# SHI-Labs/Versatile-Diffusion

Hardware: NVIDIA H100
Metric: 512x512 images/sec @ 50-step DDIM (bs=4/GPU) (higher is better)
Workload: dtype bf16

## Files before the change

versatile-diffusion_b200/csrc/attention.cu:

```cuda
#include "common.cuh"
#include "host_util.h"

namespace vdb {

constexpr int kBQ = 128;
constexpr float kRescaleThreshold = 8.0f;

struct alignas(64) AttnParams {
  CUtensorMap tmQ;
  CUtensorMap tmK;
  CUtensorMap tmV;
  int Nq, Nk;
  int q_bs, kv_bs;
  int q_col0, k_col0;
  int dv;
  int causal;
  float scale_log2;
  __nv_bfloat16* out;
  long long ldo;
  const int* kv_len;
};

template <int DK, int DVP, int BKV, int KV_STAGES>
constexpr size_t attention_smem_bytes() {
  return (DK / 64) * kBQ * 128 + KV_STAGES * ((DK / 64) * BKV * 128 + (BKV / 64) * DVP * 128) + (1 + 4 * KV_STAGES) * 8 + 1024;
}

template <int DK, int DVP, int BKV, int KV_STAGES, bool VARLEN = false>
__global__ void __launch_bounds__(288, 1) attention_kernel(const __grid_constant__ AttnParams p) {
  constexpr int KA = DK / 64;
  constexpr int KVA = BKV / 64;
  constexpr uint32_t kQBytes = KA * kBQ * 128;
  constexpr uint32_t kKBytes = KA * BKV * 128;
  constexpr uint32_t kVAtom = DVP * 128;
  constexpr uint32_t kVBytes = KVA * kVAtom;
  static_assert(BKV == 64 || BKV == 128, "kv tile");
  static_assert(kVAtom % 1024 == 0, "V atom must keep 1024B alignment");
  static_assert(DVP % 16 == 0 && DVP <= 256, "invalid wgmma N for PV");

  extern __shared__ __align__(1024) uint8_t smem_raw[];
  uint8_t* smem = reinterpret_cast<uint8_t*>((reinterpret_cast<uintptr_t>(smem_raw) + 1023) & ~uintptr_t(1023));
  uint8_t* sQ = smem;
  uint8_t* sK = sQ + kQBytes;
  uint8_t* sV = sK + KV_STAGES * kKBytes;
  uint64_t* q_full = reinterpret_cast<uint64_t*>(sV + KV_STAGES * kVBytes);
  uint64_t* k_full = q_full + 1;
  uint64_t* k_empty = k_full + KV_STAGES;
  uint64_t* v_full = k_empty + KV_STAGES;
  uint64_t* v_empty = v_full + KV_STAGES;

  const int warp = threadIdx.x >> 5;
  const int lane = threadIdx.x & 31;
  const int q0 = blockIdx.x * kBQ;
  const int head = blockIdx.y;
  const int b = blockIdx.z;

  int nk = 0;
  int ntiles = (p.Nk + BKV - 1) / BKV;
  if (p.causal) ntiles = min(ntiles, (q0 + kBQ + BKV - 1) / BKV);

  if (warp == 8 && lane == 0) {
    tma_prefetch_desc(&p.tmQ);
    tma_prefetch_desc(&p.tmK);
    tma_prefetch_desc(&p.tmV);
  }
  if (threadIdx.x == 0) {
    mbar_init(q_full, 1);
    for (int s = 0; s < KV_STAGES; ++s) {
      mbar_init(&k_full[s], 1); mbar_init(&k_empty[s], 8);
      mbar_init(&v_full[s], 1); mbar_init(&v_empty[s], 8);
    }
    fence_barrier_init();
  }
  __syncthreads();
  pdl_launch_dependents();
  pdl_wait();
  if constexpr (VARLEN) {
    nk = max(0, min(p.kv_len[b], p.Nk));
    ntiles = (nk + BKV - 1) / BKV;
  }

  if (warp == 8) {
    if (lane == 0) {
      mbar_arrive_expect_tx(q_full, kQBytes);
      for (int a = 0; a < KA; ++a)
        tma_load_2d(sQ + a * kBQ * 128, &p.tmQ, q_full, p.q_col0 + head * DK + a * 64, b * p.q_bs + q0);
      for (int j = 0; j < ntiles; ++j) {
        const int st = j % KV_STAGES;
        const uint32_t ph = (j / KV_STAGES) & 1;
        mbar_wait(&k_empty[st], ph ^ 1);
        mbar_arrive_expect_tx(&k_full[st], kKBytes);
        for (int a = 0; a < KA; ++a)
          tma_load_2d(sK + st * kKBytes + a * BKV * 128, &p.tmK, &k_full[st], p.k_col0 + head * DK + a * 64,
                      b * p.kv_bs + j * BKV);
        mbar_wait(&v_empty[st], ph ^ 1);
        mbar_arrive_expect_tx(&v_full[st], kVBytes);
        for (int a = 0; a < KVA; ++a)
          tma_load_2d(sV + st * kVBytes + a * kVAtom, &p.tmV, &v_full[st], b * p.kv_bs + j * BKV + a * 64, head * DVP);
      }
    }
    return;
  }

  const int g = warp >> 2;
  const int row0 = g * 64 + (warp & 3) * 16 + (lane >> 2);
  const int c2 = 2 * (lane & 3);
  const int q_idx[2] = {q0 + row0, q0 + row0 + 8};
  const int ksteps = (p.dv + 15) / 16;
  float o[DVP / 2];
#pragma unroll
  for (int i = 0; i < DVP / 2; ++i) o[i] = 0.f;
  float m_ref[2] = {-INFINITY, -INFINITY};
  float l_sum[2] = {0.f, 0.f};
  mbar_wait(q_full, 0);
#pragma unroll 1
  for (int j = 0; j < ntiles; ++j) {
    const int st = j % KV_STAGES;
    const uint32_t ph = (j / KV_STAGES) & 1;
    float s[BKV / 2];
    mbar_wait(&k_full[st], ph);
    wgmma_fence();
#pragma unroll
    for (int a = 0; a < KA; ++a) {
      const uint64_t qd = make_desc_sw128(smem_u32(sQ + a * kBQ * 128 + g * 64 * 128));
      const uint64_t kd = make_desc_sw128(smem_u32(sK + st * kKBytes + a * BKV * 128));
#pragma unroll
      for (int k = 0; k < 4; ++k)
        if (a * 4 + k < ksteps)
          wgmma_ss<BKV>(s, qd + 2 * k, kd + 2 * k, (a > 0 || k > 0) ? 1u : 0u);
    }
    wgmma_commit();
    wgmma_wait<0>();
    wgmma_fence_regs(s);
    __syncwarp();
    if (lane == 0) mbar_arrive(&k_empty[st]);

    const int kv0 = j * BKV;
    if (kv0 + BKV > (VARLEN ? nk : p.Nk) || p.causal) {
#pragma unroll
      for (int i = 0; i < 2; ++i) {
        const int lim = p.causal ? min(p.Nk, q_idx[i] + 1) : (VARLEN ? nk : p.Nk);
#pragma unroll
        for (int jj = 0; jj < BKV / 8; ++jj)
#pragma unroll
          for (int e = 0; e < 2; ++e)
            if (kv0 + 8 * jj + c2 + e >= lim) s[4 * jj + 2 * i + e] = -INFINITY;
      }
    }
    float m_scaled[2];
#pragma unroll
    for (int i = 0; i < 2; ++i) {
      float mx = -INFINITY;
#pragma unroll
      for (int jj = 0; jj < BKV / 8; ++jj) mx = fmaxf(mx, fmaxf(s[4 * jj + 2 * i], s[4 * jj + 2 * i + 1]));
      mx = fmaxf(mx, __shfl_xor_sync(0xffffffffu, mx, 1));
      mx = fmaxf(mx, __shfl_xor_sync(0xffffffffu, mx, 2));
      const float m_new = fmaxf(m_ref[i], mx);
      if (j == 0 || m_ref[i] == -INFINITY) {
        m_ref[i] = m_new;
      } else if ((m_new - m_ref[i]) * p.scale_log2 > kRescaleThreshold) {
        const float factor = ex2_mufu((m_ref[i] - m_new) * p.scale_log2);
        m_ref[i] = m_new;
        l_sum[i] *= factor;
#pragma unroll
        for (int jj = 0; jj < DVP / 8; ++jj) {
          o[4 * jj + 2 * i] *= factor;
          o[4 * jj + 2 * i + 1] *= factor;
        }
      }
      m_scaled[i] = (m_ref[i] == -INFINITY) ? 0.f : m_ref[i] * p.scale_log2;
    }
    uint32_t pa[BKV / 16][4];
#pragma unroll
    for (int kk = 0; kk < BKV / 16; ++kk) {
#pragma unroll
      for (int h = 0; h < 4; ++h) {
        const int i = h & 1;
        const int idx = 8 * kk + 4 * (h >> 1) + 2 * i;
        const float e0 = ex2_mufu(fmaf(s[idx], p.scale_log2, -m_scaled[i]));
        const float e1 = ex2_mufu(fmaf(s[idx + 1], p.scale_log2, -m_scaled[i]));
        l_sum[i] += e0 + e1;
        pa[kk][h] = pack_bf16x2(e0, e1);
      }
    }
    mbar_wait(&v_full[st], ph);
    wgmma_fence();
#pragma unroll
    for (int kk = 0; kk < BKV / 16; ++kk) {
      const uint64_t vd = make_desc_sw128(smem_u32(sV + st * kVBytes + (kk >> 2) * kVAtom));
      wgmma_rs<DVP>(o, pa[kk], vd + 2 * (kk & 3), 1u);
    }
    wgmma_commit();
    wgmma_wait<0>();
    wgmma_fence_regs(o);
    __syncwarp();
    if (lane == 0) mbar_arrive(&v_empty[st]);
  }

#pragma unroll
  for (int i = 0; i < 2; ++i) {
    float l = l_sum[i];
    l += __shfl_xor_sync(0xffffffffu, l, 1);
    l += __shfl_xor_sync(0xffffffffu, l, 2);
    const float inv_l = (VARLEN && !(l > 0.f)) ? 0.f : 1.f / l;
    if (q_idx[i] >= p.Nq) continue;
    __nv_bfloat16* orow = p.out + (static_cast<long long>(b) * p.q_bs + q_idx[i]) * p.ldo + head * p.dv;
#pragma unroll
    for (int jj = 0; jj < DVP / 8; ++jj) {
      const int col = 8 * jj + c2;
      if (col < p.dv)
        *reinterpret_cast<uint32_t*>(orow + col) = pack_bf16x2(o[4 * jj + 2 * i] * inv_l, o[4 * jj + 2 * i + 1] * inv_l);
    }
  }
}

struct AttnArgs {
  const void *Q, *K, *Vt;
  long long ldq, ldk, ldv;
  int B, H, q_bstride, kv_bstride;
};

template <int DK, int DVP, int BKV, int KV_STAGES, bool VARLEN = false>
static int launch_attention(AttnParams& p, const AttnArgs& a, cudaStream_t stream) {
  constexpr size_t smem = attention_smem_bytes<DK, DVP, BKV, KV_STAGES>();
  static_assert(smem <= 227 * 1024, "attention smem budget");
  auto kernel = attention_kernel<DK, DVP, BKV, KV_STAGES, VARLEN>;
  static bool configured = false;
  if (!configured) {
    VDB_CUDA_CHECK(cudaFuncSetAttribute(kernel, cudaFuncAttributeMaxDynamicSharedMemorySize, static_cast<int>(smem)));
    prefer_max_smem(kernel);
    configured = true;
  }
  int rc = make_tmap_2d(&p.tmQ, a.Q, static_cast<uint64_t>(a.ldq), static_cast<uint64_t>(a.B) * a.q_bstride, a.ldq * 2, 64, kBQ);
  if (rc) return rc;
  rc = make_tmap_2d(&p.tmK, a.K, static_cast<uint64_t>(a.ldk), static_cast<uint64_t>(a.B) * a.kv_bstride, a.ldk * 2, 64, BKV);
  if (rc) return rc;
  rc = make_tmap_2d(&p.tmV, a.Vt, static_cast<uint64_t>(a.B) * a.kv_bstride, static_cast<uint64_t>(a.H) * DVP, a.ldv * 2, 64, DVP);
  if (rc) return rc;
  dim3 grid((p.Nq + kBQ - 1) / kBQ, a.H, a.B);
  VDB_CUDA_CHECK(launch_pdl(kernel, grid, dim3(288), smem, stream, p));
  count_launch();
  return VDB_OK;
}

}

using namespace vdb;

extern "C" {

int vdb_attention_dk_pad(int d_head) { return d_head <= 64 ? 64 : (d_head <= 128 ? 128 : (d_head <= 192 ? 192 : -1)); }
int vdb_attention_dv_pad(int d_head) {
  if (d_head <= 48) return 48;
  if (d_head <= 64) return 64;
  if (d_head <= 80) return 80;
  if (d_head <= 160) return 160;
  return -1;
}

static int attention_prepare(const void* Q, long long ldq, int q_col0, const void* K, long long ldk, int k_col0, const void* Vt,
                             long long ldv, void* out, long long ldo, int B, int H, int Nq, int Nk, int q_bstride, int kv_bstride,
                             int d_head, float scale, int causal, AttnParams& p, AttnArgs& a) {
  if (!Q || !K || !Vt || !out || B <= 0 || H <= 0 || Nq <= 0 || Nk <= 0)
    return set_error(VDB_ERR_INVALID, "attention: null/empty argument");
  const int DK = vdb_attention_dk_pad(d_head), DVP = vdb_attention_dv_pad(d_head);
  if (DK < 0 || DVP < 0) return set_error(VDB_ERR_UNSUPPORTED, "attention: d_head %d not supported (<= 160)", d_head);
  if ((d_head % 8) || (ldo % 8) || (ldq % 8) || (ldk % 8) || (ldv % 8))
    return set_error(VDB_ERR_INVALID, "attention: d_head and leading dims must be multiples of 8");
  if (q_bstride <= 0) q_bstride = Nq;
  if (kv_bstride <= 0) kv_bstride = Nk;
  if (q_bstride < Nq || kv_bstride < Nk || (kv_bstride % 8))
    return set_error(VDB_ERR_INVALID, "attention: need q_bstride >= Nq, kv_bstride >= Nk and kv_bstride %% 8 == 0 (got %d, %d)",
                     q_bstride, kv_bstride);
  memset(&p, 0, sizeof(p));
  a = AttnArgs{Q, K, Vt, ldq, ldk, ldv, B, H, q_bstride, kv_bstride};
  p.Nq = Nq; p.Nk = Nk; p.q_bs = q_bstride; p.kv_bs = kv_bstride; p.q_col0 = q_col0; p.k_col0 = k_col0; p.dv = d_head; p.causal = causal;
  p.scale_log2 = scale * 1.4426950408889634f;
  p.out = reinterpret_cast<__nv_bfloat16*>(out);
  p.ldo = ldo;
  return VDB_OK;
}

int vdb_attention_bf16(const void* Q, long long ldq, int q_col0, const void* K, long long ldk, int k_col0,
                       const void* Vt, long long ldv, void* out, long long ldo, int B, int H, int Nq, int Nk,
                       int q_bstride, int kv_bstride, int d_head, float scale, int causal, void* stream) {
  AttnParams p;
  AttnArgs a{};
  const int rc = attention_prepare(Q, ldq, q_col0, K, ldk, k_col0, Vt, ldv, out, ldo, B, H, Nq, Nk, q_bstride, kv_bstride, d_head,
                                   scale, causal, p, a);
  if (rc) return rc;
  const int DK = vdb_attention_dk_pad(d_head), DVP = vdb_attention_dv_pad(d_head);
  cudaStream_t st = reinterpret_cast<cudaStream_t>(stream);
  if (DK == 64 && DVP == 48) return launch_attention<64, 48, 128, 2>(p, a, st);
  if (DK == 64 && DVP == 64) return launch_attention<64, 64, 128, 2>(p, a, st);
  if (DK == 128 && DVP == 80) return launch_attention<128, 80, 128, 2>(p, a, st);
  if (DK == 192 && DVP == 160) return launch_attention<192, 160, 64, 2>(p, a, st);
  return set_error(VDB_ERR_UNSUPPORTED, "attention: no kernel for d_head %d", d_head);
}

int vdb_attention_varlen_bf16(const void* Q, long long ldq, int q_col0, const void* K, long long ldk, int k_col0,
                              const void* Vt, long long ldv, void* out, long long ldo, int B, int H, int Nq, int Nk,
                              int q_bstride, int kv_bstride, int d_head, float scale, int causal, const int* kv_len,
                              void* stream) {
  if (!kv_len || (reinterpret_cast<uintptr_t>(kv_len) & 3))
    return set_error(VDB_ERR_INVALID, "attention_varlen: kv_len must be a non-null, 4-byte aligned device int32 [B]");
  if (causal) return set_error(VDB_ERR_INVALID, "attention_varlen: causal masking together with kv_len is not supported");
  if (vdb_attention_dk_pad(d_head) != 64 || vdb_attention_dv_pad(d_head) != 64)
    return set_error(VDB_ERR_UNSUPPORTED, "attention_varlen: only d_head 64 (BERT) is instantiated, got %d", d_head);
  AttnParams p;
  AttnArgs a{};
  const int rc = attention_prepare(Q, ldq, q_col0, K, ldk, k_col0, Vt, ldv, out, ldo, B, H, Nq, Nk, q_bstride, kv_bstride, d_head,
                                   scale, causal, p, a);
  if (rc) return rc;
  p.kv_len = kv_len;
  return launch_attention<64, 64, 128, 2, true>(p, a, reinterpret_cast<cudaStream_t>(stream));
}

}
```

versatile-diffusion_b200/csrc/common.cuh:

```cuda
#pragma once
#include <cuda.h>
#include <cuda_bf16.h>
#include <cuda_runtime.h>
#include <stdint.h>

namespace vdb {

#define VDB_DEVINL __device__ __forceinline__

enum : int {
  VDB_OK = 0,
  VDB_ERR_INVALID = 1,
  VDB_ERR_CUDA = 2,
  VDB_ERR_UNSUPPORTED = 3,
};

VDB_DEVINL float4 lds_f4(uint32_t addr) {
  float4 v;
  asm volatile("ld.shared.v4.f32 {%0, %1, %2, %3}, [%4];" : "=f"(v.x), "=f"(v.y), "=f"(v.z), "=f"(v.w) : "r"(addr));
  return v;
}

VDB_DEVINL float2 lds_f2(uint32_t addr) {
  float2 v;
  asm volatile("ld.shared.v2.f32 {%0, %1}, [%2];" : "=f"(v.x), "=f"(v.y) : "r"(addr));
  return v;
}
VDB_DEVINL void stmatrix_x4(uint32_t addr, uint32_t r0, uint32_t r1, uint32_t r2, uint32_t r3) {
  asm volatile("stmatrix.sync.aligned.m8n8.x4.shared.b16 [%0], {%1, %2, %3, %4};" ::"r"(addr), "r"(r0), "r"(r1), "r"(r2), "r"(r3)
               : "memory");
}

VDB_DEVINL uint32_t smem_u32(const void* p) {
  return static_cast<uint32_t>(__cvta_generic_to_shared(p));
}

VDB_DEVINL uint32_t lane_id() {
  uint32_t l;
  asm volatile("mov.u32 %0, %%laneid;" : "=r"(l));
  return l;
}

VDB_DEVINL bool elect_one() {
  uint32_t pred = 0;
  asm volatile(
      "{\n\t"
      ".reg .pred P;\n\t"
      "elect.sync _|P, 0xffffffff;\n\t"
      "selp.u32 %0, 1, 0, P;\n\t"
      "}\n"
      : "=r"(pred));
  return pred != 0;
}

VDB_DEVINL void mbar_init(uint64_t* bar, uint32_t count) {
  asm volatile("mbarrier.init.shared::cta.b64 [%0], %1;" ::"r"(smem_u32(bar)), "r"(count));
}
VDB_DEVINL void fence_barrier_init() {
  asm volatile("fence.mbarrier_init.release.cluster;" ::: "memory");
}
VDB_DEVINL void fence_proxy_async_smem() {
  asm volatile("fence.proxy.async.shared::cta;" ::: "memory");
}
VDB_DEVINL void mbar_arrive_expect_tx(uint64_t* bar, uint32_t bytes) {
  asm volatile("mbarrier.arrive.expect_tx.shared::cta.b64 _, [%0], %1;" ::"r"(smem_u32(bar)),
               "r"(bytes)
               : "memory");
}
VDB_DEVINL void mbar_arrive(uint64_t* bar) {
  asm volatile("mbarrier.arrive.shared::cta.b64 _, [%0];" ::"r"(smem_u32(bar)) : "memory");
}
VDB_DEVINL bool mbar_try_wait(uint64_t* bar, uint32_t parity) {
  uint32_t ok;
  asm volatile(
      "{\n\t"
      ".reg .pred P;\n\t"
      "mbarrier.try_wait.parity.shared::cta.b64 P, [%1], %2;\n\t"
      "selp.u32 %0, 1, 0, P;\n\t"
      "}\n"
      : "=r"(ok)
      : "r"(smem_u32(bar)), "r"(parity)
      : "memory");
  return ok != 0;
}
VDB_DEVINL void mbar_wait(uint64_t* bar, uint32_t parity) {
  while (!mbar_try_wait(bar, parity)) {
  }
}

VDB_DEVINL void tma_prefetch_desc(const CUtensorMap* m) {
  asm volatile("prefetch.tensormap [%0];" ::"l"(reinterpret_cast<uint64_t>(m)) : "memory");
}
VDB_DEVINL void tma_load_2d(void* smem_dst, const CUtensorMap* m, uint64_t* bar, int c0, int c1) {
  asm volatile(
      "cp.async.bulk.tensor.2d.shared::cluster.global.tile.mbarrier::complete_tx::bytes"
      " [%0], [%1, {%3, %4}], [%2];" ::"r"(smem_u32(smem_dst)),
      "l"(reinterpret_cast<uint64_t>(m)), "r"(smem_u32(bar)), "r"(c0), "r"(c1)
      : "memory");
}
VDB_DEVINL void tma_load_4d(void* smem_dst, const CUtensorMap* m, uint64_t* bar, int c0, int c1,
                            int c2, int c3) {
  asm volatile(
      "cp.async.bulk.tensor.4d.shared::cluster.global.tile.mbarrier::complete_tx::bytes"
      " [%0], [%1, {%3, %4, %5, %6}], [%2];" ::"r"(smem_u32(smem_dst)),
      "l"(reinterpret_cast<uint64_t>(m)), "r"(smem_u32(bar)), "r"(c0), "r"(c1), "r"(c2), "r"(c3)
      : "memory");
}

VDB_DEVINL void tma_store_4d(const CUtensorMap* m, const void* smem_src, int c0, int c1, int c2, int c3) {
  asm volatile(
      "cp.async.bulk.tensor.4d.global.shared::cta.tile.bulk_group [%0, {%2, %3, %4, %5}], [%1];" ::"l"(
          reinterpret_cast<uint64_t>(m)),
      "r"(smem_u32(smem_src)), "r"(c0), "r"(c1), "r"(c2), "r"(c3)
      : "memory");
}
VDB_DEVINL void bulk_commit() { asm volatile("cp.async.bulk.commit_group;" ::: "memory"); }
template <int N>
VDB_DEVINL void bulk_wait_read() { asm volatile("cp.async.bulk.wait_group.read %0;" ::"n"(N) : "memory"); }
template <int N>
VDB_DEVINL void bulk_wait() { asm volatile("cp.async.bulk.wait_group %0;" ::"n"(N) : "memory"); }

VDB_DEVINL uint32_t cluster_ctarank() {
  uint32_t r;
  asm volatile("mov.u32 %0, %%cluster_ctarank;" : "=r"(r));
  return r;
}
VDB_DEVINL void cluster_sync_all() {
  asm volatile("barrier.cluster.arrive.release.aligned;\n\tbarrier.cluster.wait.acquire.aligned;" ::: "memory");
}
VDB_DEVINL uint32_t mapa_u32(uint32_t local_addr, uint32_t rank) {
  uint32_t r;
  asm volatile("mapa.shared::cluster.u32 %0, %1, %2;" : "=r"(r) : "r"(local_addr), "r"(rank));
  return r;
}
VDB_DEVINL void mbar_arrive_cluster(uint32_t cluster_addr) {
  asm volatile("mbarrier.arrive.release.cluster.shared::cluster.b64 _, [%0];" ::"r"(cluster_addr) : "memory");
}

VDB_DEVINL uint64_t make_desc_sw128(uint32_t smem_addr) {
  uint64_t d = 0;
  d |= static_cast<uint64_t>((smem_addr & 0x3FFFF) >> 4);
  d |= static_cast<uint64_t>(1) << 16;
  d |= static_cast<uint64_t>(1024 >> 4) << 32;
  d |= static_cast<uint64_t>(1) << 62;
  return d;
}
VDB_DEVINL void wgmma_fence() { asm volatile("wgmma.fence.sync.aligned;" ::: "memory"); }
VDB_DEVINL void wgmma_commit() { asm volatile("wgmma.commit_group.sync.aligned;" ::: "memory"); }
template <int N>
VDB_DEVINL void wgmma_wait() { asm volatile("wgmma.wait_group.sync.aligned %0;" ::"n"(N) : "memory"); }
template <int R>
VDB_DEVINL void wgmma_fence_regs(float (&d)[R]) {
#pragma unroll
  for (int i = 0; i < R; ++i) asm volatile("" : "+f"(d[i])::"memory");
}

VDB_DEVINL unsigned long long gtime() {
  unsigned long long t;
  asm volatile("mov.u64 %0, %%globaltimer;" : "=l"(t));
  return t;
}

VDB_DEVINL void pdl_wait() { asm volatile("griddepcontrol.wait;" ::: "memory"); }
VDB_DEVINL void pdl_launch_dependents() { asm volatile("griddepcontrol.launch_dependents;" ::: "memory"); }

VDB_DEVINL uint32_t pack_bf16x2(float lo, float hi) {
  __nv_bfloat162 v = __floats2bfloat162_rn(lo, hi);
  return *reinterpret_cast<uint32_t*>(&v);
}
VDB_DEVINL float2 unpack_bf16x2(uint32_t u) {
  __nv_bfloat162 v = *reinterpret_cast<__nv_bfloat162*>(&u);
  return __bfloat1622float2(v);
}
VDB_DEVINL float ex2_mufu(float x) {
  float y;
  asm("ex2.approx.ftz.f32 %0, %1;" : "=f"(y) : "f"(x));
  return y;
}
VDB_DEVINL float ex2_poly(float x) {
  x = fmaxf(x, -126.0f);
  const float r = x + 12582912.0f;
  const float f = x - (r - 12582912.0f);
  float p = fmaf(0.0550886838f, f, 0.242604051f);
  p = fmaf(p, f, 0.693276242f);
  p = fmaf(p, f, 0.99992894f);
  return __int_as_float(__float_as_int(p) + (__float_as_int(r) << 23));
}
VDB_DEVINL float silu_f(float x) { return __fdividef(x, 1.0f + __expf(-x)); }
VDB_DEVINL float silu_bf16_f(float x) {
  float th;
  asm("tanh.approx.f32 %0, %1;" : "=f"(th) : "f"(0.5f * x));
  const float hx = 0.5f * x;
  return fmaf(hx, th, hx);
}
VDB_DEVINL float gelu_erf_f(float x) { return 0.5f * x * (1.0f + erff(x * 0.70710678118654752f)); }
VDB_DEVINL float gelu_as_f(float x) {
  const float z = fabsf(x) * 0.70710678118654752f;
  const float t = __fdividef(1.0f, fmaf(0.3275911f, z, 1.0f));
  float poly = fmaf(1.061405429f, t, -1.453152027f);
  poly = fmaf(poly, t, 1.421413741f);
  poly = fmaf(poly, t, -0.284496736f);
  poly = fmaf(poly, t, 0.254829592f);
  const float erf_abs = 1.0f - poly * t * __expf(-z * z);
  return 0.5f * x * (1.0f + copysignf(erf_abs, x));
}
VDB_DEVINL float gelu_fast_f(float x) {
  const float u = x * fmaf(0.0356774081f, x * x, 0.7978845608f);
  float th;
  asm("tanh.approx.f32 %0, %1;" : "=f"(th) : "f"(u));
  const float hx = 0.5f * x;
  return fmaf(hx, th, hx);
}
VDB_DEVINL float quick_gelu_f(float x) { return __fdividef(x, 1.0f + __expf(-1.702f * x)); }

}

#include "wgmma.cuh"
```

Before: 4.652.

## Pipeline QK and PV wgmma across tiles with warp-specialized register reallocation

Restructures the attention consumer loop so the S=QK^T wgmma for tile j is issued together with the PV wgmma for tile j-1, with softmax overlapping the in-flight PV. The kernel grows to 384 threads: a 128-thread producer warpgroup gives up registers via setmaxnreg and two consumer warpgroups take more. It also adds a mask-free fast path for full tiles, offloads part of the exp2 work to an FMA polynomial for the DK=64/DVP=48 case, and fixes underflow handling in ex2_poly. The aim is to hide tensor-core latency behind softmax work, at the cost of higher register pressure and double-buffered P fragments. The QK k-step count is now fixed at DVP/16 instead of derived from p.dv, which looks like a semantic change.

```diff
diff --git a/versatile-diffusion_b200/csrc/attention.cu b/versatile-diffusion_b200/csrc/attention.cu
--- a/versatile-diffusion_b200/csrc/attention.cu
+++ b/versatile-diffusion_b200/csrc/attention.cu
@@ -1,3 +1,5 @@
+#include <type_traits>
+
 #include "common.cuh"
 #include "host_util.h"
 
@@ -5,6 +7,9 @@
 
 constexpr int kBQ = 128;
 constexpr float kRescaleThreshold = 8.0f;
+constexpr int kAttnThreads = 384;
+constexpr int kProducerRegs = 40;
+constexpr int kConsumerRegs = 232;
 
 struct alignas(64) AttnParams {
   CUtensorMap tmQ;
@@ -26,8 +31,12 @@
   return (DK / 64) * kBQ * 128 + KV_STAGES * ((DK / 64) * BKV * 128 + (BKV / 64) * DVP * 128) + (1 + 4 * KV_STAGES) * 8 + 1024;
 }
 
+__host__ __device__ constexpr int attention_exp2_poly_of8(int DK, int DVP) {
+  return (DK == 64 && DVP == 48) ? 1 : 0;
+}
+
 template <int DK, int DVP, int BKV, int KV_STAGES, bool VARLEN = false>
-__global__ void __launch_bounds__(288, 1) attention_kernel(const __grid_constant__ AttnParams p) {
+__global__ void __launch_bounds__(kAttnThreads, 1) attention_kernel(const __grid_constant__ AttnParams p) {
   constexpr int KA = DK / 64;
   constexpr int KVA = BKV / 64;
   constexpr uint32_t kQBytes = KA * kBQ * 128;
@@ -37,6 +46,8 @@
   static_assert(BKV == 64 || BKV == 128, "kv tile");
   static_assert(kVAtom % 1024 == 0, "V atom must keep 1024B alignment");
   static_assert(DVP % 16 == 0 && DVP <= 256, "invalid wgmma N for PV");
+  constexpr int kExp2PolyOf8 = attention_exp2_poly_of8(DK, DVP);
+  constexpr int kSSteps = DVP / 16;
 
   extern __shared__ __align__(1024) uint8_t smem_raw[];
   uint8_t* smem = reinterpret_cast<uint8_t*>((reinterpret_cast<uintptr_t>(smem_raw) + 1023) & ~uintptr_t(1023));
@@ -55,11 +66,7 @@
   const int head = blockIdx.y;
   const int b = blockIdx.z;
 
-  int nk = 0;
-  int ntiles = (p.Nk + BKV - 1) / BKV;
-  if (p.causal) ntiles = min(ntiles, (q0 + kBQ + BKV - 1) / BKV);
-
-  if (warp == 8 && lane == 0) {
+  if (warp == 0 && lane == 0) {
     tma_prefetch_desc(&p.tmQ);
     tma_prefetch_desc(&p.tmK);
     tma_prefetch_desc(&p.tmV);
@@ -75,13 +82,16 @@
   __syncthreads();
   pdl_launch_dependents();
   pdl_wait();
-  if constexpr (VARLEN) {
-    nk = max(0, min(p.kv_len[b], p.Nk));
-    ntiles = (nk + BKV - 1) / BKV;
-  }
-
-  if (warp == 8) {
-    if (lane == 0) {
+  auto key_count = [&] { return VARLEN ? max(0, min(p.kv_len[b], p.Nk)) : p.Nk; };
+  auto tile_count = [&](int nk) {
+    const int n = (nk + BKV - 1) / BKV;
+    return p.causal ? min(n, (q0 + kBQ + BKV - 1) / BKV) : n;
+  };
+
+  if (warp < 4) {
+    setmaxnreg_dec<kProducerRegs>();
+    const int ntiles = tile_count(key_count());
+    if (warp == 0 && lane == 0) {
       mbar_arrive_expect_tx(q_full, kQBytes);
       for (int a = 0; a < KA; ++a)
         tma_load_2d(sQ + a * kBQ * 128, &p.tmQ, q_full, p.q_col0 + head * DK + a * 64, b * p.q_bs + q0);
@@ -102,23 +112,26 @@
     return;
   }
 
-  const int g = warp >> 2;
+  setmaxnreg_inc<kConsumerRegs>();
+  const int nk = key_count();
+  const int ntiles = tile_count(nk);
+  const int g = (warp >> 2) - 1;
   const int row0 = g * 64 + (warp & 3) * 16 + (lane >> 2);
   const int c2 = 2 * (lane & 3);
   const int q_idx[2] = {q0 + row0, q0 + row0 + 8};
-  const int ksteps = (p.dv + 15) / 16;
   float o[DVP / 2];
 #pragma unroll
   for (int i = 0; i < DVP / 2; ++i) o[i] = 0.f;
   float m_ref[2] = {-INFINITY, -INFINITY};
   float l_sum[2] = {0.f, 0.f};
-  mbar_wait(q_full, 0);
-#pragma unroll 1
-  for (int j = 0; j < ntiles; ++j) {
+  float o_factor[2];
+  bool o_rescale[2];
+  float s[BKV / 2];
+  uint32_t pa[BKV / 16][4], pb[BKV / 16][4];
+
+  auto issue_s = [&](int j) {
     const int st = j % KV_STAGES;
-    const uint32_t ph = (j / KV_STAGES) & 1;
-    float s[BKV / 2];
-    mbar_wait(&k_full[st], ph);
+    mbar_wait(&k_full[st], (j / KV_STAGES) & 1);
     wgmma_fence();
 #pragma unroll
     for (int a = 0; a < KA; ++a) {
@@ -126,75 +139,126 @@
       const uint64_t kd = make_desc_sw128(smem_u32(sK + st * kKBytes + a * BKV * 128));
 #pragma unroll
       for (int k = 0; k < 4; ++k)
-        if (a * 4 + k < ksteps)
+        if (a * 4 + k < kSSteps)
           wgmma_ss<BKV>(s, qd + 2 * k, kd + 2 * k, (a > 0 || k > 0) ? 1u : 0u);
     }
     wgmma_commit();
-    wgmma_wait<0>();
-    wgmma_fence_regs(s);
+  };
+  auto issue_pv = [&](int j, const uint32_t(&pp)[BKV / 16][4]) {
+    const int st = j % KV_STAGES;
+    mbar_wait(&v_full[st], (j / KV_STAGES) & 1);
+    wgmma_fence();
+#pragma unroll
+    for (int kk = 0; kk < BKV / 16; ++kk) {
+      const uint64_t vd = make_desc_sw128(smem_u32(sV + st * kVBytes + (kk >> 2) * kVAtom));
+      wgmma_rs<DVP>(o, pp[kk], vd + 2 * (kk & 3), 1u);
+    }
+    wgmma_commit();
+  };
+  auto release = [&](uint64_t* empty, int j) {
     __syncwarp();
-    if (lane == 0) mbar_arrive(&k_empty[st]);
-
+    if (lane == 0) mbar_arrive(&empty[j % KV_STAGES]);
+  };
+  auto softmax_tile = [&](int j, uint32_t(&pp)[BKV / 16][4], auto masked) {
+    constexpr bool kMasked = decltype(masked)::value;
     const int kv0 = j * BKV;
-    if (kv0 + BKV > (VARLEN ? nk : p.Nk) || p.causal) {
-#pragma unroll
-      for (int i = 0; i < 2; ++i) {
-        const int lim = p.causal ? min(p.Nk, q_idx[i] + 1) : (VARLEN ? nk : p.Nk);
-#pragma unroll
-        for (int jj = 0; jj < BKV / 8; ++jj)
-#pragma unroll
-          for (int e = 0; e < 2; ++e)
-            if (kv0 + 8 * jj + c2 + e >= lim) s[4 * jj + 2 * i + e] = -INFINITY;
-      }
-    }
+    int lim[2];
+#pragma unroll
+    for (int i = 0; i < 2; ++i) lim[i] = p.causal ? min(p.Nk, q_idx[i] + 1) : (VARLEN ? nk : p.Nk);
+    auto sv = [&](int jj, int i, int e) {
+      const float v = s[4 * jj + 2 * i + e];
+      if constexpr (kMasked) return (kv0 + 8 * jj + c2 + e >= lim[i]) ? -INFINITY : v;
+      return v;
+    };
     float m_scaled[2];
 #pragma unroll
     for (int i = 0; i < 2; ++i) {
       float mx = -INFINITY;
 #pragma unroll
-      for (int jj = 0; jj < BKV / 8; ++jj) mx = fmaxf(mx, fmaxf(s[4 * jj + 2 * i], s[4 * jj + 2 * i + 1]));
+      for (int jj = 0; jj < BKV / 8; ++jj) mx = fmaxf(mx, fmaxf(sv(jj, i, 0), sv(jj, i, 1)));
       mx = fmaxf(mx, __shfl_xor_sync(0xffffffffu, mx, 1));
       mx = fmaxf(mx, __shfl_xor_sync(0xffffffffu, mx, 2));
       const float m_new = fmaxf(m_ref[i], mx);
+      o_rescale[i] = false;
       if (j == 0 || m_ref[i] == -INFINITY) {
         m_ref[i] = m_new;
       } else if ((m_new - m_ref[i]) * p.scale_log2 > kRescaleThreshold) {
         const float factor = ex2_mufu((m_ref[i] - m_new) * p.scale_log2);
         m_ref[i] = m_new;
         l_sum[i] *= factor;
+        o_factor[i] = factor;
+        o_rescale[i] = true;
+      }
+      m_scaled[i] = (m_ref[i] == -INFINITY) ? 0.f : m_ref[i] * p.scale_log2;
+    }
+#pragma unroll
+    for (int kk = 0; kk < BKV / 16; ++kk) {
+#pragma unroll
+      for (int h = 0; h < 4; ++h) {
+        const int i = h & 1;
+        const int jj = 2 * kk + (h >> 1);
+        const float x0 = fmaf(sv(jj, i, 0), p.scale_log2, -m_scaled[i]);
+        const float x1 = fmaf(sv(jj, i, 1), p.scale_log2, -m_scaled[i]);
+        const bool fma_pipe = ((4 * kk + h) & 7) < kExp2PolyOf8;
+        const float e0 = fma_pipe ? ex2_poly(x0) : ex2_mufu(x0);
+        const float e1 = fma_pipe ? ex2_poly(x1) : ex2_mufu(x1);
+        l_sum[i] += e0 + e1;
+        pp[kk][h] = pack_bf16x2(e0, e1);
+      }
+    }
+  };
+  auto softmax = [&](int j, uint32_t(&pp)[BKV / 16][4]) {
+    if ((j + 1) * BKV > (VARLEN ? nk : p.Nk) || p.causal)
+      softmax_tile(j, pp, std::true_type{});
+    else
+      softmax_tile(j, pp, std::false_type{});
+  };
+  auto step = [&](int j, const uint32_t(&p_prev)[BKV / 16][4], uint32_t(&p_cur)[BKV / 16][4]) {
+    issue_s(j);
+    issue_pv(j - 1, p_prev);
+    wgmma_wait<1>();
+    wgmma_fence_regs(s);
+    release(k_empty, j);
+    softmax(j, p_cur);
+    wgmma_wait<0>();
+    wgmma_fence_regs(o);
+    release(v_empty, j - 1);
+#pragma unroll
+    for (int i = 0; i < 2; ++i)
+      if (o_rescale[i]) {
 #pragma unroll
         for (int jj = 0; jj < DVP / 8; ++jj) {
-          o[4 * jj + 2 * i] *= factor;
-          o[4 * jj + 2 * i + 1] *= factor;
+          o[4 * jj + 2 * i] *= o_factor[i];
+          o[4 * jj + 2 * i + 1] *= o_factor[i];
         }
       }
-      m_scaled[i] = (m_ref[i] == -INFINITY) ? 0.f : m_ref[i] * p.scale_log2;
-    }
-    uint32_t pa[BKV / 16][4];
-#pragma unroll
-    for (int kk = 0; kk < BKV / 16; ++kk) {
-#pragma unroll
-      for (int h = 0; h < 4; ++h) {
-        const int i = h & 1;
-        const int idx = 8 * kk + 4 * (h >> 1) + 2 * i;
-        const float e0 = ex2_mufu(fmaf(s[idx], p.scale_log2, -m_scaled[i]));
-        const float e1 = ex2_mufu(fmaf(s[idx + 1], p.scale_log2, -m_scaled[i]));
-        l_sum[i] += e0 + e1;
-        pa[kk][h] = pack_bf16x2(e0, e1);
-      }
-    }
-    mbar_wait(&v_full[st], ph);
-    wgmma_fence();
-#pragma unroll
-    for (int kk = 0; kk < BKV / 16; ++kk) {
-      const uint64_t vd = make_desc_sw128(smem_u32(sV + st * kVBytes + (kk >> 2) * kVAtom));
-      wgmma_rs<DVP>(o, pa[kk], vd + 2 * (kk & 3), 1u);
-    }
-    wgmma_commit();
+  };
+  auto finish = [&](int j, const uint32_t(&p_last)[BKV / 16][4]) {
+    issue_pv(j, p_last);
     wgmma_wait<0>();
     wgmma_fence_regs(o);
-    __syncwarp();
-    if (lane == 0) mbar_arrive(&v_empty[st]);
+    release(v_empty, j);
+  };
+
+  mbar_wait(q_full, 0);
+  if (ntiles > 0) {
+    issue_s(0);
+    wgmma_wait<0>();
+    wgmma_fence_regs(s);
+    release(k_empty, 0);
+    softmax(0, pa);
+    int j = 1;
+#pragma unroll 1
+    for (; j + 1 < ntiles; j += 2) {
+      step(j, pa, pb);
+      step(j + 1, pb, pa);
+    }
+    if (j < ntiles) {
+      step(j, pa, pb);
+      finish(j, pb);
+    } else {
+      finish(j - 1, pa);
+    }
   }
 
 #pragma unroll
@@ -238,7 +302,7 @@
   rc = make_tmap_2d(&p.tmV, a.Vt, static_cast<uint64_t>(a.B) * a.kv_bstride, static_cast<uint64_t>(a.H) * DVP, a.ldv * 2, 64, DVP);
   if (rc) return rc;
   dim3 grid((p.Nq + kBQ - 1) / kBQ, a.H, a.B);
-  VDB_CUDA_CHECK(launch_pdl(kernel, grid, dim3(288), smem, stream, p));
+  VDB_CUDA_CHECK(launch_pdl(kernel, grid, dim3(kAttnThreads), smem, stream, p));
   count_launch();
   return VDB_OK;
 }
diff --git a/versatile-diffusion_b200/csrc/common.cuh b/versatile-diffusion_b200/csrc/common.cuh
--- a/versatile-diffusion_b200/csrc/common.cuh
+++ b/versatile-diffusion_b200/csrc/common.cuh
@@ -155,6 +155,11 @@
   for (int i = 0; i < R; ++i) asm volatile("" : "+f"(d[i])::"memory");
 }
 
+template <int N>
+VDB_DEVINL void setmaxnreg_dec() { asm volatile("setmaxnreg.dec.sync.aligned.u32 %0;" ::"n"(N)); }
+template <int N>
+VDB_DEVINL void setmaxnreg_inc() { asm volatile("setmaxnreg.inc.sync.aligned.u32 %0;" ::"n"(N)); }
+
 VDB_DEVINL unsigned long long gtime() {
   unsigned long long t;
   asm volatile("mov.u64 %0, %%globaltimer;" : "=l"(t));
@@ -178,13 +183,14 @@
   return y;
 }
 VDB_DEVINL float ex2_poly(float x) {
-  x = fmaxf(x, -126.0f);
-  const float r = x + 12582912.0f;
-  const float f = x - (r - 12582912.0f);
+  const float xc = fmaxf(x, -127.0f);
+  const float r = xc + 12582912.0f;
+  const float f = xc - (r - 12582912.0f);
   float p = fmaf(0.0550886838f, f, 0.242604051f);
   p = fmaf(p, f, 0.693276242f);
   p = fmaf(p, f, 0.99992894f);
-  return __int_as_float(__float_as_int(p) + (__float_as_int(r) << 23));
+  const float y = __int_as_float(__float_as_int(p) + (__float_as_int(r) << 23));
+  return x < -126.0f ? 0.0f : y;
 }
 VDB_DEVINL float silu_f(float x) { return __fdividef(x, 1.0f + __expf(-x)); }
 VDB_DEVINL float silu_bf16_f(float x) {
```

Result: faster. 4.737, median of 6 (+1.8%).

## Overlap softmax with tensor-core GEMMs via warpgroup ping-pong and deferred PV

Applied to the files above, without the earlier changes.

Restructures the flash-attention consumer loop in a FA3-style way. The PV wgmma for the previous tile is issued right after the QK^T wgmma of the current tile, so it runs while softmax is computed. Named barriers make the two consumer warpgroups take turns issuing tensor-core work, so one group's exp/softmax overlaps the other group's GEMMs. Output rescaling is deferred until after the PV wait, and ksteps becomes a compile-time constant. This adds register pressure (pa held across iterations), barrier-ordering complexity, and risk of deadlock or hazards if the turn protocol is off.

```diff
diff --git a/versatile-diffusion_b200/csrc/attention.cu b/versatile-diffusion_b200/csrc/attention.cu
--- a/versatile-diffusion_b200/csrc/attention.cu
+++ b/versatile-diffusion_b200/csrc/attention.cu
@@ -1,10 +1,15 @@
 #include "common.cuh"
 #include "host_util.h"
 
+#include <type_traits>
+
 namespace vdb {
 
 constexpr int kBQ = 128;
 constexpr float kRescaleThreshold = 8.0f;
+
+VDB_DEVINL void turn_wait(int g) { asm volatile("bar.sync %0, 256;" ::"r"(1 + g) : "memory"); }
+VDB_DEVINL void turn_pass(int g) { asm volatile("bar.arrive %0, 256;" ::"r"(2 - g) : "memory"); }
 
 struct alignas(64) AttnParams {
   CUtensorMap tmQ;
@@ -106,19 +111,38 @@
   const int row0 = g * 64 + (warp & 3) * 16 + (lane >> 2);
   const int c2 = 2 * (lane & 3);
   const int q_idx[2] = {q0 + row0, q0 + row0 + 8};
-  const int ksteps = (p.dv + 15) / 16;
+  constexpr int ksteps = DVP / 16;
+  static_assert(ksteps <= KA * 4, "DVP <= DK");
   float o[DVP / 2];
 #pragma unroll
   for (int i = 0; i < DVP / 2; ++i) o[i] = 0.f;
   float m_ref[2] = {-INFINITY, -INFINITY};
   float l_sum[2] = {0.f, 0.f};
-  mbar_wait(q_full, 0);
-#pragma unroll 1
-  for (int j = 0; j < ntiles; ++j) {
+  uint32_t pa[BKV / 16][4];
+  auto issue_pv = [&](int pst) {
+#pragma unroll
+    for (int kk = 0; kk < BKV / 16; ++kk) {
+      const uint64_t vd = make_desc_sw128(smem_u32(sV + pst * kVBytes + (kk >> 2) * kVAtom));
+      wgmma_rs<DVP>(o, pa[kk], vd + 2 * (kk & 3), 1u);
+    }
+    wgmma_commit();
+  };
+  auto release_v = [&](int pst) {
+    wgmma_fence_regs(o);
+    wgmma_fence_regs(pa);
+    __syncwarp();
+    if (lane == 0) mbar_arrive(&v_empty[pst]);
+  };
+  auto tile = [&](int j, auto first_tile) {
+    constexpr bool first = decltype(first_tile)::value;
     const int st = j % KV_STAGES;
     const uint32_t ph = (j / KV_STAGES) & 1;
+    const int pst = (j + KV_STAGES - 1) % KV_STAGES;
+    const uint32_t pph = ((j - 1) / KV_STAGES) & 1;
     float s[BKV / 2];
+    if (!first || g == 1) turn_wait(g);
     mbar_wait(&k_full[st], ph);
+    if (!first) mbar_wait(&v_full[pst], pph);
     wgmma_fence();
 #pragma unroll
     for (int a = 0; a < KA; ++a) {
@@ -130,7 +154,9 @@
           wgmma_ss<BKV>(s, qd + 2 * k, kd + 2 * k, (a > 0 || k > 0) ? 1u : 0u);
     }
     wgmma_commit();
-    wgmma_wait<0>();
+    if constexpr (!first) issue_pv(pst);
+    turn_pass(g);
+    wgmma_wait<first ? 0 : 1>();
     wgmma_fence_regs(s);
     __syncwarp();
     if (lane == 0) mbar_arrive(&k_empty[st]);
@@ -148,53 +174,72 @@
       }
     }
     float m_scaled[2];
+    float factor[2] = {1.f, 1.f};
+    bool rescale[2] = {false, false};
 #pragma unroll
     for (int i = 0; i < 2; ++i) {
-      float mx = -INFINITY;
-#pragma unroll
-      for (int jj = 0; jj < BKV / 8; ++jj) mx = fmaxf(mx, fmaxf(s[4 * jj + 2 * i], s[4 * jj + 2 * i + 1]));
+      float m4[4] = {-INFINITY, -INFINITY, -INFINITY, -INFINITY};
+#pragma unroll
+      for (int jj = 0; jj < BKV / 8; ++jj) m4[jj & 3] = fmaxf(m4[jj & 3], fmaxf(s[4 * jj + 2 * i], s[4 * jj + 2 * i + 1]));
+      float mx = fmaxf(fmaxf(m4[0], m4[1]), fmaxf(m4[2], m4[3]));
       mx = fmaxf(mx, __shfl_xor_sync(0xffffffffu, mx, 1));
       mx = fmaxf(mx, __shfl_xor_sync(0xffffffffu, mx, 2));
       const float m_new = fmaxf(m_ref[i], mx);
-      if (j == 0 || m_ref[i] == -INFINITY) {
+      if (first || m_ref[i] == -INFINITY) {
         m_ref[i] = m_new;
       } else if ((m_new - m_ref[i]) * p.scale_log2 > kRescaleThreshold) {
-        const float factor = ex2_mufu((m_ref[i] - m_new) * p.scale_log2);
+        factor[i] = ex2_mufu((m_ref[i] - m_new) * p.scale_log2);
+        rescale[i] = true;
         m_ref[i] = m_new;
-        l_sum[i] *= factor;
-#pragma unroll
-        for (int jj = 0; jj < DVP / 8; ++jj) {
-          o[4 * jj + 2 * i] *= factor;
-          o[4 * jj + 2 * i + 1] *= factor;
-        }
+        l_sum[i] *= factor[i];
       }
       m_scaled[i] = (m_ref[i] == -INFINITY) ? 0.f : m_ref[i] * p.scale_log2;
     }
-    uint32_t pa[BKV / 16][4];
 #pragma unroll
     for (int kk = 0; kk < BKV / 16; ++kk) {
 #pragma unroll
       for (int h = 0; h < 4; ++h) {
         const int i = h & 1;
         const int idx = 8 * kk + 4 * (h >> 1) + 2 * i;
-        const float e0 = ex2_mufu(fmaf(s[idx], p.scale_log2, -m_scaled[i]));
-        const float e1 = ex2_mufu(fmaf(s[idx + 1], p.scale_log2, -m_scaled[i]));
-        l_sum[i] += e0 + e1;
-        pa[kk][h] = pack_bf16x2(e0, e1);
-      }
-    }
-    mbar_wait(&v_full[st], ph);
+        s[idx] = ex2_mufu(fmaf(s[idx], p.scale_log2, -m_scaled[i]));
+        s[idx + 1] = ex2_mufu(fmaf(s[idx + 1], p.scale_log2, -m_scaled[i]));
+        l_sum[i] += s[idx] + s[idx + 1];
+      }
+    }
+    if constexpr (!first) {
+      wgmma_wait<0>();
+      release_v(pst);
+    }
+#pragma unroll
+    for (int i = 0; i < 2; ++i)
+      if (rescale[i]) {
+#pragma unroll
+        for (int jj = 0; jj < DVP / 8; ++jj) {
+          o[4 * jj + 2 * i] *= factor[i];
+          o[4 * jj + 2 * i + 1] *= factor[i];
+        }
+      }
+#pragma unroll
+    for (int kk = 0; kk < BKV / 16; ++kk)
+#pragma unroll
+      for (int h = 0; h < 4; ++h) {
+        const int idx = 8 * kk + 4 * (h >> 1) + 2 * (h & 1);
+        pa[kk][h] = pack_bf16x2(s[idx], s[idx + 1]);
+      }
+  };
+  mbar_wait(q_full, 0);
+  if (ntiles > 0) {
+    tile(0, std::true_type{});
+#pragma unroll 1
+    for (int j = 1; j < ntiles; ++j) tile(j, std::false_type{});
+    const int pst = (ntiles - 1) % KV_STAGES;
+    turn_wait(g);
+    mbar_wait(&v_full[pst], ((ntiles - 1) / KV_STAGES) & 1);
     wgmma_fence();
-#pragma unroll
-    for (int kk = 0; kk < BKV / 16; ++kk) {
-      const uint64_t vd = make_desc_sw128(smem_u32(sV + st * kVBytes + (kk >> 2) * kVAtom));
-      wgmma_rs<DVP>(o, pa[kk], vd + 2 * (kk & 3), 1u);
-    }
-    wgmma_commit();
+    issue_pv(pst);
+    if (g == 0) turn_pass(g);
     wgmma_wait<0>();
-    wgmma_fence_regs(o);
-    __syncwarp();
-    if (lane == 0) mbar_arrive(&v_empty[st]);
+    release_v(pst);
   }
 
 #pragma unroll
diff --git a/versatile-diffusion_b200/csrc/common.cuh b/versatile-diffusion_b200/csrc/common.cuh
--- a/versatile-diffusion_b200/csrc/common.cuh
+++ b/versatile-diffusion_b200/csrc/common.cuh
@@ -153,6 +153,13 @@
 VDB_DEVINL void wgmma_fence_regs(float (&d)[R]) {
 #pragma unroll
   for (int i = 0; i < R; ++i) asm volatile("" : "+f"(d[i])::"memory");
+}
+template <int K, int R>
+VDB_DEVINL void wgmma_fence_regs(uint32_t (&a)[K][R]) {
+#pragma unroll
+  for (int k = 0; k < K; ++k)
+#pragma unroll
+    for (int i = 0; i < R; ++i) asm volatile("" : "+r"(a[k][i])::"memory");
 }
 
 VDB_DEVINL unsigned long long gtime() {
```

Result: no change. 4.553 before, 4.585 after, median of 6 (+0.7%).
